# broadinstitute/delphy

Hardware: AMD Instinct MI355X
Metric: MCMC moves/sec on 100k-tip SARS-CoV-2 EMAT at 1/2/4/8 MI355X (higher is better)
Workload: dtype f64; 1 GPU; C4: synthetic 100000-tip EMAT, 29903 sites, HKY(kappa=5) + skygrid, 8092 partition parts (199999 nodes), 1000 moves/part/step, move mix 7.5/7.5/15/1/1; parts_per_gpu=8092, parts_requested=8192, max_part_nodes=-1, lds_staging=True, tickets_per_part_and_pass=4, parallelism=parts sharded over 1 GPU(s), one wavefront per part, collectives=none (one rank), emat_build_id=7d9b3896ecee7423

## Files before the change

delphy_amd/csrc/emat_device_core.hpp:

```cpp
#ifndef EMAT_DEV_NS
#error "define EMAT_DEV_NS and EMAT_VARIANT_LDS before including the device headers"
#endif

#include <hip/hip_runtime.h>
#include <cfloat>
#include <cstdint>

#include "emat_slab.hpp"

#ifndef EMAT_DEVICE_COMMON_ONCE_
#define EMAT_DEVICE_COMMON_ONCE_
namespace emat {
extern __shared__ __attribute__((aligned(16))) uint8_t emat_lds[];
constexpr uint32_t k_lds_tables_bytes = k_max_lds_partitions * (1 + 4 + 16) * 8;
constexpr uint32_t k_lds_ctx_bytes = 288;
#ifndef EMAT_RNG_BLOCKS
#define EMAT_RNG_BLOCKS 32
#endif
constexpr uint32_t k_rng_blocks = EMAT_RNG_BLOCKS;
static_assert(k_rng_blocks == 0 || (k_rng_blocks <= 64 && (k_rng_blocks & (k_rng_blocks - 1)) == 0), "one block per lane, a power of two");
constexpr uint32_t k_lds_rng_bytes = k_rng_blocks * 16;
constexpr uint32_t k_lds_static_bytes = k_lds_tables_bytes + k_lds_ctx_bytes + k_lds_rng_bytes + k_max_lds_partitions * 16 * 8;
__shared__ __attribute__((aligned(16))) uint8_t emat_lds_tables[k_lds_tables_bytes];
__shared__ __attribute__((aligned(16))) uint8_t emat_lds_ctx[k_lds_ctx_bytes];
// ... 497 lines not shown
  double r;
  { EMAT_TIMED(0);
    r = delta_lambda_across_node_missations_fresh(c, node); }
  *e = (uint64_t)__double_as_longlong(r);
  return r;
}
template <bool kMemo = true> EMAT_D double delta_lambda_across_branch(Ctx& c, int node) {
  double r = 0.0;
  const MutRec* m = muts_of(c, node); int nm = nmuts(c, node);
  for (int i = 0; i < nm; ++i) { int l = m[i].site; r += mu_of(c)[site_part(c, l)] * site_nu(c, l) * (q_a(c, l, m[i].to) - q_a(c, l, m[i].from)); }
  r += kMemo ? delta_lambda_across_node_missations(c, node) : delta_lambda_across_node_missations_fresh(c, node);
  return r;
}
EMAT_DN double calc_lambda_at_node(Ctx& c, int node) {
  double r = c.cumQ[c.L];
  for (int cur = node; cur != k_no_node; cur = nodes_of(c)[cur].parent) r += delta_lambda_across_branch(c, cur);
  return r;
}
EMAT_D double log_mu_nu_q(const Ctx& c, int l, int a, int b) {
  const int pa = site_part(c, l); const double nu = site_nu(c, l);
  if (c.have_logq && nu == 1.0) return emat_lds_logq[pa * 16 + a * 4 + b];
  return m_log(mu_of(c)[pa] * nu * q_of(c)[pa * 16 + a * 4 + b]);
}
EMAT_D double branch_log_G(const Ctx& c, double t_P, double t_X, double lambda_X, const MutRec* m, int nm) {
  double r = -lambda_X * (t_X - t_P);
  for (int i = nm - 1; i >= 0; --i) {
    int l = m[i].site;
    r -= mu_of(c)[site_part(c, l)] * site_nu(c, l) * (q_a(c, l, m[i].from) - q_a(c, l, m[i].to)) * (m[i].t - t_P);
    r += log_mu_nu_q(c, l, m[i].from, m[i].to);
  }
  return r;
}
EMAT_DN int calc_site_state_at(Ctx& c, int branch, double t, int l) {
  for (int cur = branch; cur != k_no_node; cur = nodes_of(c)[cur].parent) {
    const MutRec* m = muts_of(c, cur);
    for (int i = nmuts(c, cur) - 1; i >= 0; --i) { if (m[i].t > t) continue; if (m[i].site == l) return m[i].to; }
  }
  return c.ref[l];
}
EMAT_D bool is_site_missing_at(Ctx& c, int node, int l) {
  for (int cur = node; cur != k_no_node; cur = nodes_of(c)[cur].parent) if (miss_contains(c, cur, l)) return true;
  return false;
}
EMAT_DN SVec<IvRec> reconstruct_missing_sites_at(Ctx& c, int node) { EMAT_TIMED(0);
  int total = 0;
  for (int cur = node; cur != k_no_node; cur = nodes_of(c)[cur].parent) total += (int)nodes_of(c)[cur].miss.cnt;
  SVec<IvRec> a = sc_vec<IvRec>(c, total + 1), b = sc_vec<IvRec>(c, total + 1);
  if (c.failed) return a;
  IvRec* so_far = a.p; IvRec* other = b.p; int n = 0;
  for (int cur = node; cur != k_no_node; cur = nodes_of(c)[cur].parent) {
    const int cnt = (int)nodes_of(c)[cur].miss.cnt;
    if (cnt == 0) continue;
    int k = iv_merge(other, so_far, n, miss_of(c, cur), cnt);
    IvRec* t = so_far; so_far = other; other = t; n = k;
  }
  SVec<IvRec> r; r.p = so_far; r.n = n; r.cap = total + 1;
  return r;
}
EMAT_D bool descends_from(Ctx& c, int X, int A) {
  if (A == k_no_node) return true;
  for (int cur = X; cur != k_no_node; cur = nodes_of(c)[cur].parent) {
    if (cur == A) return true;
    if (nodes_of(c)[cur].t < nodes_of(c)[A].t) return false;
  }
  return false;
}
EMAT_DN int find_MRCA_of(Ctx& c, int P, int Q) {
  if (P == k_no_node) return P;
  if (Q == k_no_node) return Q;
  int guard = 0;
  while (P != Q && guard++ < (1 << 28)) {
    double tP = nodes_of(c)[P].t, tQ = nodes_of(c)[Q].t;
    if (tP > tQ) { P = nodes_of(c)[P].parent; EMAT_CHECK(c, P != k_no_node); if (P == k_no_node) return Q; }
    else if (tP < tQ) { Q = nodes_of(c)[Q].parent; EMAT_CHECK(c, Q != k_no_node); if (Q == k_no_node) return P; }
    else if (is_tip(c, P)) { P = nodes_of(c)[P].parent; if (P == k_no_node) return Q; }
    else if (is_tip(c, Q)) { Q = nodes_of(c)[Q].parent; if (Q == k_no_node) return P; }
    else {
      int dP = 0, dQ = 0;
      for (int x = P; x != k_no_node; x = nodes_of(c)[x].parent) ++dP;
      for (int x = Q; x != k_no_node; x = nodes_of(c)[x].parent) ++dQ;
      int a = P, b = Q;
      while (dP > dQ) { a = nodes_of(c)[a].parent; --dP; }
      while (dQ > dP) { b = nodes_of(c)[b].parent; --dQ; }
      while (a != b) { a = nodes_of(c)[a].parent; b = nodes_of(c)[b].parent; }
      return a;
    }
  }
  return P;
}

EMAT_DF int skygrid_interval(const PopTable& p, double t) {
  const int n = p.skygrid_num_knots;
  double g = (t - p.skygrid_x[0]) * p.skygrid_inv_dx;
  int k = g > 0.0 ? (g < (double)n ? (int)g : n) : 0;
  while (k > 0 && !(p.skygrid_x[k - 1] < t)) --k;
  while (k < n && p.skygrid_x[k] < t) ++k;
  return k;
}
EMAT_DF double skygrid_log_N(const PopTable& p, double t) {
  int k = skygrid_interval(p, t), M = p.skygrid_num_knots - 1;
  if (k == 0) return p.skygrid_gamma[0];
  if (k > M) return p.skygrid_gamma[M];
  if (p.skygrid_type == 1) return p.skygrid_gamma[k];
  double cc = (t - p.skygrid_x[k - 1]) / (p.skygrid_x[k] - p.skygrid_x[k - 1]);
  return (1 - cc) * p.skygrid_gamma[k - 1] + cc * p.skygrid_gamma[k];
}
EMAT_DF double pop_at_time(const PopTable& p, double t) {
  if (p.kind == 0) return p.p[0];
  if (p.kind == 1) { double v = p.p[1] * m_exp((t - p.p[0]) * p.p[2]); return p.p[3] > v ? p.p[3] : v; }
  return m_exp(skygrid_log_N(p, t));
}
EMAT_DF double uniform_f64(double v) {
  const uint64_t a = __builtin_bit_cast(uint64_t, v);
  const uint32_t lo = __builtin_amdgcn_readfirstlane((uint32_t)a), hi = __builtin_amdgcn_readfirstlane((uint32_t)(a >> 32));
  return __builtin_bit_cast(double, ((uint64_t)hi << 32) | lo);
}
EMAT_DF double skygrid_log_N_uniform(const EMAT_CONST_AS PopTable* p, double t) {
  const EMAT_CONST_AS double* x = uniform_const_ptr((const double*)p->skygrid_x);
  const EMAT_CONST_AS double* ga = uniform_const_ptr((const double*)p->skygrid_gamma);
  const int n = p->skygrid_num_knots, M = n - 1;
  const double g = (t - x[0]) * p->skygrid_inv_dx;
  int k = __builtin_amdgcn_readfirstlane(g > 0.0 ? (g < (double)n ? (int)g : n) : 0);
  while (k > 0 && !(x[k - 1] < t)) --k;
  while (k < n && x[k] < t) ++k;
  if (k == 0) return ga[0];
  if (k > M) return ga[M];
  if (p->skygrid_type == 1) return ga[k];
  const double cc = (t - x[k - 1]) / (x[k] - x[k - 1]);
  return (1 - cc) * ga[k - 1] + cc * ga[k];
}
EMAT_DF double log_pop_ratio_uniform(const PopTable* pp, double t_new, double t_old) {
  const EMAT_CONST_AS PopTable* p = uniform_const_ptr(pp);
  const int kind = p->kind;
  if (kind == 0) return 0.0;
  t_new = uniform_f64(t_new); t_old = uniform_f64(t_old);
  if (kind == 2) return skygrid_log_N_uniform(p, t_new) - skygrid_log_N_uniform(p, t_old);
  const double t0 = p->p[0], n0 = p->p[1], gr = p->p[2], floor_n = p->p[3];
  double a = n0 * m_exp((t_new - t0) * gr); a = floor_n > a ? floor_n : a;
  double b = n0 * m_exp((t_old - t0) * gr); b = floor_n > b ? floor_n : b;
  return m_log(a / b);
}
EMAT_D double exp_unclamped_int(const PopTable& p, double a, double b) { double n0 = p.p[1], g = p.p[2], t0 = p.p[0]; return n0 / g * m_exp(g * (a - t0)) * m_expm1(g * (b - a)); }
EMAT_DN double skygrid_log_int_N(const PopTable& p, double a, double b) {
  const double* x = p.skygrid_x; const double* ge = p.skygrid_gamma;
  int M = p.skygrid_num_knots - 1;
  int ka = skygrid_interval(p, a), kb = skygrid_interval(p, b);
  int kka = ka - 1 > 0 ? ka - 1 : 0, kkb = kb < M ? kb : M;
  double bias = -k_inf;
  for (int k = kka; k <= kkb; ++k) bias = bias > ge[k] ? bias : ge[k];
  double result = 0.0;
  for (int k = ka; k <= kb; ++k) {
    double lo = k > 0 ? (a > x[k - 1] ? a : x[k - 1]) : a;
    double hi = k <= M ? (b < x[k] ? b : x[k]) : b;
    if (k == 0) result += m_exp(-bias + ge[0]) * (hi - lo);
    else if (k == M + 1) result += m_exp(-bias + ge[M]) * (hi - lo);
    else if (p.skygrid_type == 1) result += m_exp(-bias + ge[k]) * (hi - lo);
    else if (ge[k] == ge[k - 1]) result += m_exp(-bias + ge[k]) * (hi - lo);
    else {
      double c_lo = (lo - x[k - 1]) / (x[k] - x[k - 1]), c_hi = (hi - x[k - 1]) / (x[k] - x[k - 1]);
      double G_lo = (1 - c_lo) * ge[k - 1] + c_lo * ge[k], G_hi = (1 - c_hi) * ge[k - 1] + c_hi * ge[k];
      double D = G_hi - G_lo;
      if (D == 0.0) result += m_exp(-bias + G_lo) * (hi - lo);
      else result += m_exp(-bias + G_lo) * (hi - lo) * (m_expm1(D) / D);
    }
  }
  return m_log(result) + bias;
}
EMAT_NOTAIL EMAT_DN double pop_integral(const PopTable& p, double a, double b) {
  if (p.kind == 0) return (b - a) * p.p[0];
  if (p.kind == 1) {
    double n0 = p.p[1], g = p.p[2], t0 = p.p[0], min_pop = p.p[3], t_c = p.t_c;
    if (min_pop == 0.0) return g == 0.0 ? (b - a) * n0 : exp_unclamped_int(p, a, b);
    if (g == 0.0) return (b - a) * (min_pop > n0 ? min_pop : n0);
    if (g > 0.0) {
      if (b <= t_c) return (b - a) * min_pop;
      if (a >= t_c) return exp_unclamped_int(p, a, b);
      return (t_c - a) * min_pop + n0 / g * m_exp(g * (t_c - t0)) * m_expm1(g * (b - t_c));
    }
    if (a >= t_c) return (b - a) * min_pop;
    if (b <= t_c) return exp_unclamped_int(p, a, b);
    return n0 / g * m_exp(g * (a - t0)) * m_expm1(g * (t_c - a)) + (b - t_c) * min_pop;
  }
  return m_exp(skygrid_log_int_N(p, a, b));
}
EMAT_D double exp_unclamped_intensity(const PopTable& p, double a, double b) { double n0 = p.p[1], g = p.p[2], t0 = p.p[0]; return -1.0 / (n0 * g) * m_exp(-g * (a - t0)) * m_expm1(-g * (b - a)); }
EMAT_DN double skygrid_log_int_inv_N(const PopTable& p, double a, double b) {
  const double* x = p.skygrid_x; const double* gm = p.skygrid_gamma;
  int M = p.skygrid_num_knots - 1;
  int ka = skygrid_interval(p, a), kb = skygrid_interval(p, b);
  int kka = ka - 1 > 0 ? ka - 1 : 0, kkb = kb < M ? kb : M;
  double bias = -k_inf;
  for (int k = kka; k <= kkb; ++k) bias = bias > -gm[k] ? bias : -gm[k];
  double result = 0.0;
  for (int k = ka; k <= kb; ++k) {
    double lo = k > 0 ? (a > x[k - 1] ? a : x[k - 1]) : a;
    double hi = k <= M ? (b < x[k] ? b : x[k]) : b;
    if (k == 0) result += m_exp(-bias + -gm[0]) * (hi - lo);
    else if (k == M + 1) result += m_exp(-bias + -gm[M]) * (hi - lo);
    else if (p.skygrid_type == 1) result += m_exp(-bias + -gm[k]) * (hi - lo);
    else if (gm[k] == gm[k - 1]) result += m_exp(-bias + -gm[k]) * (hi - lo);
    else {
      double c_lo = (lo - x[k - 1]) / (x[k] - x[k - 1]), c_hi = (hi - x[k - 1]) / (x[k] - x[k - 1]);
      double G_lo = (1 - c_lo) * -gm[k - 1] + c_lo * -gm[k], G_hi = (1 - c_hi) * -gm[k - 1] + c_hi * -gm[k];
      double D = G_hi - G_lo;
      if (D == 0.0) result += m_exp(-bias + G_lo) * (hi - lo);
      else result += m_exp(-bias + G_lo) * (hi - lo) * (m_expm1(D) / D);
    }
  }
  return m_log(result) + bias;
}
EMAT_NOTAIL EMAT_DN double pop_intensity_integral(const PopTable& p, double a, double b) {
  if (p.kind == 0) return (b - a) / p.p[0];
  if (p.kind == 1) {
    double n0 = p.p[1], g = p.p[2], t0 = p.p[0], min_pop = p.p[3], t_c = p.t_c;
    if (min_pop == 0.0) return g == 0.0 ? (b - a) / n0 : exp_unclamped_intensity(p, a, b);
    if (g == 0.0) return (b - a) / (min_pop > n0 ? min_pop : n0);
    double inv_min_pop = 1.0 / min_pop;
    if (g > 0.0) {
      if (b <= t_c) return (b - a) * inv_min_pop;
      if (a >= t_c) return exp_unclamped_intensity(p, a, b);
      return (t_c - a) * inv_min_pop - 1.0 / (n0 * g) * m_exp(-g * (t_c - t0)) * m_expm1(-g * (b - t_c));
    }
    if (a >= t_c) return (b - a) * inv_min_pop;
    if (b <= t_c) return exp_unclamped_intensity(p, a, b);
    return -1.0 / (n0 * g) * m_exp(-g * (a - t0)) * m_expm1(-g * (t_c - a)) + (b - t_c) * inv_min_pop;
  }
  return m_exp(skygrid_log_int_inv_N(p, a, b));
}

struct Cells {
  double* kbar_p; double* ktw_p;
  double* ktw; double* popsize; double* ts_over_pop; int32_t* nactive;
  const EMAT_CONST_AS double* sh_ktw; const EMAT_CONST_AS double* sh_tsop; const EMAT_CONST_AS int32_t* sh_nact;
  int first; bool local;
};
EMAT_D Cells cells_of(Ctx& c) {
  Cells k; const int cap = hdr_of(c)->cell_cap;
  double* base = (double*)slab_at(c, hdr_of(c)->off_cells);
  k.kbar_p = base; k.ktw_p = base + cap; k.first = hdr_of(c)->cell_first; k.local = c.includes_run_root;
  if (k.local) { k.ktw = base + 2 * cap; k.popsize = base + 3 * cap; k.ts_over_pop = base + 4 * cap; k.nactive = (int32_t*)(base + 5 * cap); k.sh_ktw = nullptr; k.sh_tsop = nullptr; k.sh_nact = nullptr; }
  else { k.ktw = nullptr; k.popsize = nullptr; k.ts_over_pop = nullptr; k.nactive = nullptr; k.sh_ktw = uniform_const_ptr(c.sh_ktw); k.sh_tsop = uniform_const_ptr(c.sh_tsop); k.sh_nact = uniform_const_ptr(c.sh_nact); }
  return k;
}
EMAT_D int cell_for(const Ctx& c, double t) { return (int)floor((hdr_of(c)->t_ref - t) / hdr_of(c)->t_step); }
EMAT_D double cell_ubound(const Ctx& c, int cell) { return hdr_of(c)->t_ref - hdr_of(c)->t_step * cell; }
EMAT_D double cell_lbound(const Ctx& c, int cell) { return cell_ubound(c, cell) - hdr_of(c)->t_step; }
EMAT_NOTAIL EMAT_DN void coal_grow(Ctx& c, int cell);
template <bool kGrow = true> EMAT_DF void coal_ensure_space(Ctx& c, double t) {
  int cell = cell_for(c, t);
  if (kGrow) { if (cell >= hdr_of(c)->n_cells_total && c.includes_run_root) coal_grow(c, cell); }
  if (cell < hdr_of(c)->cell_first || cell >= hdr_of(c)->n_cells_total) EMAT_FAIL(c, k_part_internal);
}
EMAT_NOTAIL EMAT_DN void coal_grow(Ctx& c, int cell) {
  {
    Cells k = cells_of(c);
    while (hdr_of(c)->n_cells_total <= cell) {
      int i = hdr_of(c)->n_cells_total, w = i - hdr_of(c)->cell_first;
      if (w >= hdr_of(c)->cell_cap) { EMAT_FAIL(c, k_part_cell_overflow); return; }
      double popsize_bar_i = pop_integral(*c.pop, cell_lbound(c, i), cell_ubound(c, i)) / hdr_of(c)->t_step;
      double sigma = sqrt(popsize_bar_i / hdr_of(c)->t_step);
      double ktw = gaussian(c, 0.0, sigma);
      k.popsize[w] = popsize_bar_i; k.ts_over_pop[w] = hdr_of(c)->t_step / popsize_bar_i; k.nactive[w] = 1; k.kbar_p[w] = 1.0; k.ktw_p[w] = ktw; k.ktw[w] = ktw;
      hdr_of(c)->n_cells_total = i + 1; hdr_of(c)->n_cells = w + 1;
    }
  }
}
EMAT_DF bool coal_needs_cells(const Ctx& c, double t) {
  if (!c.includes_run_root) return false;
  const int cell = cell_for(c, t);
  return cell >= hdr_of(c)->n_cells_total && cell - hdr_of(c)->cell_first >= hdr_of(c)->cell_cap;
}
EMAT_DN void stop_for_cells(Ctx& c, int kind) {
  rng_rewind_to_move_start(c);
  hdr_of(c)->proposed[kind]--;
  c.failed = true;
  if (hdr_of(c)->status == 0) hdr_of(c)->status = k_part_need_cells;
}
EMAT_DF void coal_add_interval(Ctx& c, double t_start, double t_end, double delta_k) {
  if (c.failed) return;
  if (t_start < t_end) { double t = t_start; t_start = t_end; t_end = t; }
  Cells k = cells_of(c);
  const int first = hdr_of(c)->cell_first;
  int cell_start = cell_for(c, t_start);
  int cell_end = hdr_of(c)->n_cells_total - 1;
  if (t_end != cell_lbound(c, cell_end)) cell_end = cell_for(c, t_end);
  if (cell_start < first || cell_end >= hdr_of(c)->n_cells_total || cell_start > cell_end) { EMAT_FAIL(c, k_part_internal); return; }
  const double ts = hdr_of(c)->t_step;
  if (cell_start == cell_end) k.kbar_p[cell_start - first] += delta_k * (t_start - t_end) / ts;
  else {
    k.kbar_p[cell_start - first] += delta_k * (t_start - cell_lbound(c, cell_start)) / ts;
    k.kbar_p[cell_end - first] += delta_k * (cell_ubound(c, cell_end) - t_end) / ts;
    for (int i = cell_start + 1; i < cell_end; ++i) k.kbar_p[i - first] += delta_k;
  }
  c.bytes += 8 * (int64_t)(cell_end - cell_start + 1); c.bytes_w += 8 * (int64_t)(cell_end - cell_start + 1);
}
EMAT_DF double coal_cell_term(const Ctx& c, const Cells& k, int w, double new_k, double old_k) {
  double na, tsop, ktw;
  if (k.local) { na = (double)k.nactive[w]; tsop = k.ts_over_pop[w]; ktw = k.ktw[w]; }
  else { const int i = __builtin_amdgcn_readfirstlane(k.first + w); na = (double)k.sh_nact[i]; tsop = k.sh_tsop[i]; ktw = k.sh_ktw[i]; }
  return tsop * (
      +0.5 * (new_k * new_k - old_k * old_k) * na
      - (k.ktw_p[w] * na - ktw + 0.5) * (new_k - old_k));
}
template <bool kGrow = true> EMAT_DF double coal_delta_on_add_interval(Ctx& c, double min_t, double max_t, double delta_k) { EMAT_TIMED(0);
  { int cm = cell_for(c, max_t); if (cm < hdr_of(c)->cell_first || cm >= hdr_of(c)->n_cells_total) { EMAT_FAIL(c, k_part_internal); return 0.0; } }
  coal_ensure_space<kGrow>(c, min_t);
  if (c.failed) return 0.0;
  if (min_t == max_t) return 0.0;
  Cells k = cells_of(c);
  const int first = hdr_of(c)->cell_first; const double ts = hdr_of(c)->t_step;
  int cell_start = cell_for(c, max_t), cell_end = cell_for(c, min_t);
  double d = 0.0;
  if (cell_start == cell_end) {
    int w = cell_start - first;
    double old_k = k.kbar_p[w], new_k = old_k + delta_k * (max_t - min_t) / ts;
    d -= coal_cell_term(c, k, w, new_k, old_k);
  } else {
    int i = cell_start;
    double dt_start = max_t - cell_lbound(c, cell_start);
    double dt_end = cell_ubound(c, cell_end) - min_t;
    double old_k = k.kbar_p[i - first], new_k = old_k + delta_k * dt_start / ts;
    d -= coal_cell_term(c, k, i - first, new_k, old_k);
    for (++i; i < cell_end; ++i) { old_k = k.kbar_p[i - first]; new_k = old_k + delta_k; d -= coal_cell_term(c, k, i - first, new_k, old_k); }
    old_k = k.kbar_p[i - first]; new_k = old_k + delta_k * dt_end / ts;
    d -= coal_cell_term(c, k, i - first, new_k, old_k);
  }
  c.bytes += 36 * (int64_t)(cell_end - cell_start + 1);
  EMAT_COUNT(c, 13, cell_end - cell_start + 1); EMAT_COUNT(c, 14, 1);
  return d;
}
template <bool kGrow = true> EMAT_DF double coal_delta_displace_coalescence(Ctx& c, double old_t, double new_t) { EMAT_TIMED(0);
  double d = (old_t <= new_t) ? coal_delta_on_add_interval<kGrow>(c, old_t, new_t, -1.0) : coal_delta_on_add_interval<kGrow>(c, new_t, old_t, +1.0);
  { EMAT_TIMED(0); d -= log_pop_ratio_uniform(c.pop, new_t, old_t); }
  return d;
}
template <bool kGrow = true> EMAT_DF double coal_delta_displace_tip(Ctx& c, double old_t, double new_t) {
  return (old_t <= new_t) ? coal_delta_on_add_interval<kGrow>(c, old_t, new_t, +1.0) : coal_delta_on_add_interval<kGrow>(c, new_t, old_t, -1.0);
}
template <bool kGrow = true> EMAT_DF void coal_coalescence_displaced(Ctx& c, double old_t, double new_t) {
  coal_ensure_space<kGrow>(c, new_t);
  coal_add_interval(c, old_t, new_t, old_t <= new_t ? -1.0 : +1.0);
}
template <bool kGrow = true> EMAT_DF void coal_tip_displaced(Ctx& c, double old_t, double new_t) {
  coal_ensure_space<kGrow>(c, new_t);
  coal_add_interval(c, old_t, new_t, old_t <= new_t ? +1.0 : -1.0);
}

EMAT_DN double gamma_q_fraction(double a, double x) {
  const double FPMIN = 1e-300;
  double b = x + 1.0 - a, cc = 1.0 / FPMIN, d = 1.0 / b, h = d;
  for (int i = 1; i < 100000; ++i) {
    double an = -i * (i - a);
    b += 2.0;
    d = an * d + b; if (fabs(d) < FPMIN) d = FPMIN;
    cc = b + an / cc; if (fabs(cc) < FPMIN) cc = FPMIN;
    d = 1.0 / d;
    double del = d * cc; h *= del;
    if (fabs(del - 1.0) < 1e-16) break;
  }
  return h;
}
EMAT_DN double gamma_q(double a, double x) {
  if (x == 0.0) return 1.0;
  if (isinf(x)) return 0.0;
  const double lg = lgamma(a);
  if (x < a + 1.0) {
    double ap = a, sum = 1.0 / a, del = sum;
    for (int n = 0; n < 100000; ++n) { ap += 1.0; del *= x / ap; sum += del; if (fabs(del) < fabs(sum) * 1e-17) break; }
    return 1.0 - sum * m_exp(-x + a * m_log(x) - lg);
  }
  return m_exp(-x + a * m_log(x) - lg) * gamma_q_fraction(a, x);
}
EMAT_DN double gamma_q_inv(double a, double q) {
  if (q == 0.0) return k_inf;
  if (q == 1.0) return 0.0;
  const double lg = lgamma(a);
  if (q < 1e-3) {
    const double lq = m_log(q);
    double x = a + 1.0, h = gamma_q_fraction(a, x), prev = 0.0;
    if (-x + a * m_log(x) - lg + m_log(h) > lq) {
      for (int j = 0; j < 100; ++j) {
        double dx = (-x + a * m_log(x) - lg + m_log(h) - lq) * x * h;
        double xn = x + dx;
        if (xn < a + 1.0) xn = a + 1.0;
        bool done = fabs(xn - x) <= 1e-14 * xn || (j > 2 && fabs(dx) >= fabs(prev));
        x = xn; prev = dx;
        if (done) break;
        h = gamma_q_fraction(a, x);
      }
      return x;
    }
  }
  const double p = 1.0 - q;
  double x;
  if (a > 1.0) {
    double pp = (p < 0.5) ? p : q;
    double t = sqrt(-2.0 * m_log(pp));
    double xg = (2.30753 + t * 0.27061) / (1.0 + t * (0.99229 + t * 0.04481)) - t;
    if (p < 0.5) xg = -xg;
    double v = a * pow(1.0 - 1.0 / (9.0 * a) - xg / (3.0 * sqrt(a)), 3.0);
    x = v > 1e-3 ? v : 1e-3;
  } else {
    double t = 1.0 - a * (0.253 + a * 0.12);
    if (p < t) x = pow(p / t, 1.0 / a);
    else x = 1.0 - m_log(1.0 - (p - t) / (1.0 - t));
  }
  const double a1 = a - 1.0;
  for (int j = 0; j < 60; ++j) {
    if (x <= 0.0) x = 1e-300;
    double err = gamma_q(a, x) - q;
    double tdens = m_exp(-x + a1 * m_log(x) - lg);
    if (tdens == 0.0) break;
    double u = -err / tdens;
    double w = u * (a1 / x - 1.0);
    double dx = u / (1.0 - 0.5 * (w < 1.0 ? w : 1.0));
    double xn = x - dx;
    if (xn <= 0.0) xn = 0.5 * x;
    double tol = 1e-15 * (xn > 1e-300 ? xn : 1e-300);
    if (fabs(xn - x) < tol) { x = xn; break; }
    x = xn;
  }
  return x;
}

}
}
```

delphy_amd/csrc/emat_device_moves.hpp:

```cpp

#include "emat_device_spr.hpp"

namespace emat {
namespace EMAT_DEV_NS {

#ifndef EMAT_HOT_BYTES
#define EMAT_HOT_BYTES 1536
#endif
enum { k_inner_node_displace = 0, k_tip_displace = 1, k_branch_reform = 2, k_subtree_slide = 3, k_spr1 = 4 };

EMAT_D void begin_move(Ctx& c, int kind) { hdr_of(c)->proposed[kind]++; c.tr_kind = (double)kind; c.tr_node = -1.0; c.tr_acc = 0.0; c.tr_log_mh = __builtin_nan(""); }
EMAT_D void note_move(Ctx& c, int node, double log_mh, bool acc, int kind) { c.tr_node = (double)node; c.tr_log_mh = log_mh; c.tr_acc = acc ? 1.0 : 0.0; if (acc) hdr_of(c)->accepted[kind]++; }
EMAT_D bool mh_accept(Ctx& c, double log_mh) { return log_mh >= 0.0 || uniform_co(c, 0.0, 1.0) < m_exp(log_mh); }

EMAT_DF double bounded_exponential(Ctx& c, double lambda, double a, double b) {
  double u = u01_oo(c);
  double ltr = lambda * (b - a);
  double x;
  if (lambda == 0.0) x = a + u * (b - a);
  else if (lambda > 0 && ltr > 100) x = b + m_log(u) / lambda;
  else if (lambda < 0 && ltr < -100) x = a + m_log(u) / lambda;
  else x = a + m_log1p(u * (m_exp(ltr) - 1)) / lambda;
  return x < a ? a : (b < x ? b : x);
}
EMAT_DF int pick_random_node(Ctx& c) { return uniform_int(c, hdr_of(c)->n_nodes); }

struct CoreFrame {
  int X, new_branch, P, old_S;
  double new_t, alpha_ratio, old_t_P, d_prior, log_mh;
  Graft old_graft, new_graft;
};
#ifndef EMAT_CF
#define EMAT_CF(c) (*(CoreFrame*)(c).frame)
#endif
EMAT_NOTAIL EMAT_DN void spr_move_core(Ctx& c, int X, int new_branch, double new_t, double alpha_ratio) { EMAT_TIMED(2);
  if (X == hdr_of(c)->root) return;
  if (!c.includes_run_root) if (nodes_of(c)[X].parent == hdr_of(c)->root || new_branch == hdr_of(c)->root) return;
  {
    const double t_X = nodes_of(c)[X].t;
    const int P = nodes_of(c)[X].parent;
    const double new_t_P = new_t;
    if (new_t_P == t_X || new_t_P == nodes_of(c)[new_branch].t || (P != hdr_of(c)->root && new_t_P == nodes_of(c)[nodes_of(c)[P].parent].t)) return;
    if (coal_needs_cells(c, new_t_P)) { stop_for_cells(c, (int)c.tr_kind); return; }
    CoreFrame* f = (CoreFrame*)sc_alloc(c, (uint32_t)sizeof(CoreFrame));
    if (c.failed) return;
    c.frame = (uint8_t*)f;
    f->X = X; f->new_branch = new_branch; f->P = P; f->old_S = sibling_of(c, P, X);
    f->new_t = new_t; f->alpha_ratio = alpha_ratio; f->old_t_P = nodes_of(c)[P].t;
  }
  c.mu_prop = nodes_of(c)[hdr_of(c)->root].lambda / (c.L - nodes_of(c)[hdr_of(c)->root].n_missing);
  EMAT_PHASE_BEGIN();
  analyze_graft(c, EMAT_CF(c).X, EMAT_CF(c).old_graft);
  peel_graft(c, EMAT_CF(c).old_graft);
  EMAT_PHASE(c, 0);
  spr_move_topology(c, EMAT_CF(c).X, EMAT_CF(c).new_branch, EMAT_CF(c).new_t);
  EMAT_PHASE(c, 1);
  propose_new_graft(c, EMAT_CF(c).X, EMAT_CF(c).new_graft);
  EMAT_PHASE(c, 2);
  if (c.failed) return;
  EMAT_CF(c).d_prior = coal_delta_displace_coalescence(c, EMAT_CF(c).old_t_P, EMAT_CF(c).new_t);
  {
    const CoreFrame& f = EMAT_CF(c);
    EMAT_CF(c).log_mh = (f.new_graft.delta_log_G - f.new_graft.log_alpha_mut) - (f.old_graft.delta_log_G - f.old_graft.log_alpha_mut) + m_log(f.alpha_ratio) + f.d_prior;
  }
  if (c.failed) return;
  const bool acc = mh_accept(c, EMAT_CF(c).log_mh);
  if (c.tr_kind == (double)k_subtree_slide) note_move(c, EMAT_CF(c).X, EMAT_CF(c).log_mh, acc, k_subtree_slide);
  if (acc) {
    apply_graft(c, EMAT_CF(c).new_graft);
    hdr_of(c)->log_G -= EMAT_CF(c).old_graft.delta_log_G; hdr_of(c)->log_G += EMAT_CF(c).new_graft.delta_log_G;
    hdr_of(c)->log_aug_prior += EMAT_CF(c).d_prior;
    coal_coalescence_displaced(c, EMAT_CF(c).old_t_P, EMAT_CF(c).new_t);
  } else {
    spr_move_topology(c, EMAT_CF(c).X, EMAT_CF(c).old_S, EMAT_CF(c).old_t_P);
    apply_graft(c, EMAT_CF(c).old_graft);
  }
  EMAT_PHASE(c, 4);
}

template <bool kRoot> EMAT_NOTAIL EMAT_DN void inner_node_displace_move(Ctx& c) { EMAT_TIMED(2);
  begin_move(c, k_inner_node_displace);
  int node;
  { EMAT_TIMED(2);
    int guard = 0; do { node = pick_random_node(c); } while (is_tip(c, node) && guard++ < (1 << 26)); }
  c.tr_node = (double)node;
  const int root = hdr_of(c)->root;
  if (!kRoot && node == root) return;
  const NodeRec nd = nodes_of(c)[node];
  double t_min = -k_inf;
  if (!kRoot || node != root) {
    t_min = nodes_of(c)[nd.parent].t;
    const MutRec* m = muts_of(c, node);
    for (int i = 0; i < (int)nd.muts.cnt; ++i) t_min = t_min > m[i].t ? t_min : m[i].t;
  }
  double t_max = k_inf;
  const int ch[2] = {nd.child0, nd.child1};
  const double lambda_at_node = nd.lambda;
  double d_logG_dt = 0.0;
  if (!kRoot || node != root) d_logG_dt += -lambda_at_node;
  for (int k = 0; k < 2; ++k) {
    const int cc = ch[k];
    t_max = t_max < nodes_of(c)[cc].t ? t_max : nodes_of(c)[cc].t;
    const MutRec* m = muts_of(c, cc);
    const int nm = nmuts(c, cc);
    for (int i = 0; i < nm; ++i) t_max = t_max < m[i].t ? t_max : m[i].t;
    c.bytes += 64 + 16 * nm + 24 * (int)nodes_of(c)[cc].miss.cnt;
  }
  { EMAT_TIMED(2);
  for (int k = 0; k < 2; ++k) {
    double lambda_just_below = lambda_at_node + delta_lambda_across_node_missations(c, ch[k]);
    d_logG_dt -= -lambda_just_below;
  } }
  c.bytes += 2 * 64 + 16 * (int)nd.muts.cnt;
  const double old_t = nd.t;
  double log_alpha_ratio = 0.0, new_t = old_t;
  if (kRoot && node == root) {
    double tree_span = c.t_max_tip - t_max;
    EMAT_CHECK(c, tree_span >= 0.0);
    double ds = (1 / nd.lambda) / 2;
    double delta_scale;
    if (tree_span < ds) delta_scale = tree_span; else delta_scale = ds;
    new_t = old_t + gaussian(c, 0.0, delta_scale);
    if (new_t < t_min || new_t > t_max) return;
    log_alpha_ratio = 0.0;
  } else {
    EMAT_TIMED(2);
    new_t = bounded_exponential(c, d_logG_dt, t_min, t_max);
    log_alpha_ratio = d_logG_dt * (new_t - old_t);
  }
  if (new_t == t_min || new_t == t_max) return;
  if (kRoot) { if (coal_needs_cells(c, new_t)) { stop_for_cells(c, k_inner_node_displace); return; } }
  double delta_log_G = d_logG_dt * (new_t - old_t);
  double delta_log_prior = coal_delta_displace_coalescence<kRoot>(c, old_t, new_t);
  if (c.failed) return;
  double log_mh = delta_log_G + delta_log_prior - log_alpha_ratio;
  bool acc;
  { EMAT_TIMED(2);
  acc = mh_accept(c, log_mh);
  note_move(c, node, log_mh, acc, k_inner_node_displace); }
  if (acc) {
    EMAT_TIMED(2);
    coal_coalescence_displaced<kRoot>(c, old_t, new_t);
    nodes_of(c)[node].t = new_t;
    hdr_of(c)->log_G += d_logG_dt * (new_t - old_t);
    hdr_of(c)->log_aug_prior += delta_log_prior;
  }
}

template <bool kRoot> EMAT_NOTAIL EMAT_DN void tip_displace_move(Ctx& c) { EMAT_TIMED(2);
  begin_move(c, k_tip_displace);
  int node;
  { int guard = 0; do { node = pick_random_node(c); } while (!is_tip(c, node) && guard++ < (1 << 26)); }
  c.tr_node = (double)node;
  const NodeRec nd = nodes_of(c)[node];
  if (nd.t_min == nd.t_max) return;
  double t_min;
  if ((double)nd.t_min < nodes_of(c)[nd.parent].t) t_min = nodes_of(c)[nd.parent].t; else t_min = (double)nd.t_min;
  const MutRec* m = muts_of(c, node);
  for (int i = 0; i < (int)nd.muts.cnt; ++i) t_min = t_min > m[i].t ? t_min : m[i].t;
  const double t_max = (double)nd.t_max;
  const double d_logG_dt = -nd.lambda;
  const double old_t = nd.t;
  c.bytes += 2 * 64 + 16 * (int)nd.muts.cnt;
  double new_t = bounded_exponential(c, d_logG_dt, t_min, t_max);
  double log_alpha_ratio = d_logG_dt * (new_t - old_t);
  if (new_t == t_min || new_t == t_max) return;
  double delta_log_G = d_logG_dt * (new_t - old_t);
  double delta_log_prior = coal_delta_displace_tip<kRoot>(c, old_t, new_t);
  if (c.failed) return;
  double log_mh = delta_log_G + delta_log_prior - log_alpha_ratio;
  bool acc = mh_accept(c, log_mh);
  note_move(c, node, log_mh, acc, k_tip_displace);
  if (acc) {
    coal_tip_displaced<kRoot>(c, old_t, new_t);
    nodes_of(c)[node].t = new_t;
    hdr_of(c)->log_G += d_logG_dt * (new_t - old_t);
    hdr_of(c)->log_aug_prior += delta_log_prior;
  }
}

EMAT_DF SVec<MutRec> randomize_branch_mutation_times(Ctx& c, int X) { EMAT_TIMED(2);
  const int n = nmuts(c, X);
  SVec<MutRec> out = sc_vec<MutRec>(c, n);
  if (c.failed) return out;
  const MutRec* old = muts_of(c, X);
  if (X == hdr_of(c)->root) { for (int i = 0; i < n; ++i) push(c, out, old[i]); return out; }
  const double t_X = nodes_of(c)[X].t, t_P = nodes_of(c)[nodes_of(c)[X].parent].t;
  bool complicated = false;
  for (int i = 0; i < n && !complicated; ++i) for (int j = i + 1; j < n; ++j) if (old[i].site == old[j].site) { complicated = true; break; }
  if (!complicated) {
    for (int i = 0; i < n; ++i) { MutRec r = make_mut(old[i].from, old[i].site, old[i].to, uniform_oc(c, t_P, t_X)); r.pad = (uint16_t)i; push(c, out, r); }
  } else {
    int prev_site = -1;
    while (true) {
      int l = 0x7fffffff;
      for (int i = 0; i < n; ++i) if (old[i].site > prev_site && old[i].site < l) l = old[i].site;
      if (l == 0x7fffffff) break;
      prev_site = l;
      int first = out.n, k = 0;
      for (int i = 0; i < n; ++i) if (old[i].site == l) { MutRec r = make_mut(old[i].from, old[i].site, old[i].to, uniform_oc(c, t_P, t_X)); r.pad = (uint16_t)i; push(c, out, r); ++k; }
      for (int a = first + 1; a < first + k && a < out.n; ++a) { double x = out.p[a].t; int b = a - 1; while (b >= first && out.p[b].t > x) { out.p[b + 1].t = out.p[b].t; --b; } out.p[b + 1].t = x; }
    }
  }
  sort_muts(out.p, out.n);
  return out;
}

struct ReformFactors { double* A; double* B; };
EMAT_DF ReformFactors reform_factors(Ctx& c, const MutRec* m, int n) { EMAT_TIMED(2);
  ReformFactors f; f.A = (double*)sc_alloc(c, (uint32_t)n * 16u); f.B = f.A + n;
  if (c.failed) return f;
  uint32_t need_log = 0u; bool all_logs = false;
  for (int j0 = 0; j0 < n; j0 += 4) {
    int l[4]; int pa[4]; double nu[4];
#pragma unroll
    for (int k = 0; k < 4; ++k) l[k] = m[j0 + k < n ? j0 + k : n - 1].site;
#pragma unroll
    for (int k = 0; k < 4; ++k) { pa[k] = site_part(c, l[k]); nu[k] = site_nu(c, l[k]); }
#pragma unroll
    for (int k = 0; k < 4; ++k) if (j0 + k < n) {
      const MutRec& mm = m[j0 + k];
      const double mn = mu_of(c)[pa[k]] * nu[k];
      const double* q = q_of(c) + pa[k] * 16;
      f.A[j0 + k] = mn * (-q[(int)mm.from * 5] - -q[(int)mm.to * 5]);
      if (c.have_logq && nu[k] == 1.0) f.B[j0 + k] = emat_lds_logq[pa[k] * 16 + (int)mm.from * 4 + (int)mm.to];
      else { f.B[j0 + k] = mn * q[(int)mm.from * 4 + (int)mm.to]; need_log |= 1u << ((j0 + k) & 31); if (j0 + k >= 32) all_logs = true; }
    }
  }
  if (all_logs) { for (int j = 0; j < n; ++j) if (!(c.have_logq && site_nu(c, m[j].site) == 1.0)) f.B[j] = m_log(f.B[j]); }
  else if (need_log != 0u) { const int n32 = n < 32 ? n : 32; for (int j = 0; j < n32; ++j) if ((need_log >> j) & 1u) f.B[j] = m_log(f.B[j]); }
  return f;
}
template <bool kRoot> EMAT_NOTAIL EMAT_DN void branch_reform_move(Ctx& c) { EMAT_TIMED(2);
  begin_move(c, k_branch_reform);
  if (hdr_of(c)->n_nodes < 3) return;
  const int X = pick_random_node(c);
  c.tr_node = (double)X;
  if (X == hdr_of(c)->root) return;
  const int P = nodes_of(c)[X].parent;
  const int S = sibling_of(c, P, X);
  const double t_X = nodes_of(c)[X].t, t_P = nodes_of(c)[P].t;
  if (kRoot) { if (P == hdr_of(c)->root) { spr_move_core(c, X, S, t_P, 1.0); if (c.failed) return; } }
  const double lam = nodes_of(c)[X].lambda;
  const int n = nmuts(c, X);
  if (n == 0) {
    const double g = -lam * (t_X - t_P), delta_log_G = g - g;
    c.bytes += 2 * 64;
    const bool acc = mh_accept(c, delta_log_G);
    note_move(c, X, delta_log_G, acc, k_branch_reform);
    if (acc) hdr_of(c)->log_G += delta_log_G;
    return;
  }
  const ReformFactors f = reform_factors(c, muts_of(c, X), n);
  SVec<MutRec> nm = randomize_branch_mutation_times(c, X);
  if (c.failed) return;
  double g_new = -lam * (t_X - t_P), g_old = g_new;
  { const MutRec* m = nm.p; for (int i = nm.n - 1; i >= 0; --i) { const int j = (int)m[i].pad; g_new -= f.A[j] * (m[i].t - t_P); g_new += f.B[j]; } }
  { const MutRec* m = muts_of(c, X); for (int i = n - 1; i >= 0; --i) { g_old -= f.A[i] * (m[i].t - t_P); g_old += f.B[i]; } }
  const double delta_log_G = g_new - g_old;
  c.bytes += 2 * 64 + 2 * 16 * nm.n;
  double log_mh = delta_log_G;
  bool acc = mh_accept(c, log_mh);
  note_move(c, X, log_mh, acc, k_branch_reform);
  if (acc) {
    for (int i = 0; i < nm.n; ++i) nm.p[i].pad = 0;
    list_assign<MutRec>(c, nodes_of(c)[X].muts, nm.p, nm.n); hdr_of(c)->log_G += delta_log_G; c.bytes += 16 * nm.n; c.bytes_w += 16 * nm.n;
  }
}

EMAT_DN SVec<int> enumerate_descendant_branches_straddling(Ctx& c, int P, double t, int X) {
  SVec<int> out; out.n = 0;
  ScSpan span = sc_span(c, 512);
  out.p = (int*)span.lo; out.cap = 0;
  int* stack_base = (int*)span.hi;
  int sp = 0;
  auto room = [&](int er, int es) -> bool {
    if (span.lo + (size_t)(out.n + er) * 4 + 16 <= span.hi - (size_t)(sp + es) * 4) return true;
    if (!span.lds) return false;
    ScSpan big = sc_span_hbm(c);
    if (big.lo + (size_t)(out.n + er) * 4 + 16 > big.hi - (size_t)(sp + es) * 4) return false;
    int* no = (int*)big.lo; int* nb = (int*)big.hi;
    for (int i = 0; i < out.n; ++i) no[i] = out.p[i];
    for (int i = 1; i <= sp; ++i) nb[-i] = stack_base[-i];
    span = big; out.p = no; stack_base = nb;
    return true;
  };
  if (!room(0, 1)) { EMAT_FAIL(c, k_part_overflow); return out; }
  stack_base[-(++sp)] = P;
  while (sp > 0 && !c.failed) {
    int n = stack_base[-sp]; --sp;
    if (n == X) continue;
    if (t <= nodes_of(c)[n].t) { if (!room(1, 0)) { EMAT_FAIL(c, k_part_overflow); break; } out.p[out.n++] = n; }
    else if (!is_tip(c, n)) {
      if (!room(0, 2)) { EMAT_FAIL(c, k_part_overflow); break; }
      stack_base[-(++sp)] = nodes_of(c)[n].child1;
      stack_base[-(++sp)] = nodes_of(c)[n].child0;
    }
  }
  out.cap = out.n;
  sc_span_commit(c, span, (uint32_t)out.n * 4u);
  return out;
}

EMAT_NOTAIL EMAT_DN void subtree_slide_move(Ctx& c) { EMAT_TIMED(2);
  begin_move(c, k_subtree_slide);
  if (hdr_of(c)->n_nodes < 2) return;
  const int X = pick_random_node(c);
  c.tr_node = (double)X;
  const int root = hdr_of(c)->root;
  if (X == root) return;
  const int P = nodes_of(c)[X].parent, S = sibling_of(c, P, X);
  double t_early = (P == root) ? (nodes_of(c)[X].t < nodes_of(c)[S].t ? nodes_of(c)[X].t : nodes_of(c)[S].t) : nodes_of(c)[root].t;
  if (P == root) { if (nodes_of(c)[S].t < nodes_of(c)[X].t) t_early = nodes_of(c)[S].t; else t_early = nodes_of(c)[X].t; }
  double tree_span = c.t_max_tip - t_early;
  EMAT_CHECK(c, tree_span >= 0.0);
  double ds = (1 / nodes_of(c)[X].lambda) / 2;
  double delta_scale = tree_span < ds ? tree_span : ds;
  double delta_t = gaussian(c, 0.0, delta_scale);
  const double old_P_t = nodes_of(c)[P].t, new_P_t = old_P_t + delta_t;
  if (delta_t < 0.0) {
    if (P != root && new_P_t < nodes_of(c)[nodes_of(c)[P].parent].t) {
      int GG = nodes_of(c)[P].parent, SS = P;
      while (new_P_t < nodes_of(c)[GG].t) { SS = GG; GG = nodes_of(c)[GG].parent; if (GG == k_no_node) break; }
      SVec<int> branches = enumerate_descendant_branches_straddling(c, SS, old_P_t, X);
      if (c.failed) return;
      double a_o2n = 1.0, a_n2o = 1.0 / (double)branches.n;
      spr_move_core(c, X, SS, new_P_t, a_n2o / a_o2n);
    } else spr_move_core(c, X, S, new_P_t, 1.0);
  } else {
    if (new_P_t > nodes_of(c)[X].t) return;
    if (new_P_t > nodes_of(c)[S].t) {
      SVec<int> branches = enumerate_descendant_branches_straddling(c, P, new_P_t, X);
      if (c.failed) return;
      if (branches.n == 0) return;
      int bi = uniform_int(c, branches.n);
      int SS = branches.p[bi];
      double a_o2n = 1.0 / (double)branches.n, a_n2o = 1.0;
      spr_move_core(c, X, SS, new_P_t, a_n2o / a_o2n);
    } else spr_move_core(c, X, S, new_P_t, 1.0);
  }
}

EMAT_D void spr1_park(Ctx& c, int phase) { c.phase = (uint8_t)phase; c.svc = 1; }
EMAT_NOTAIL EMAT_DN void spr1_move_begin(Ctx& c) { EMAT_TIMED(2);
  begin_move(c, k_spr1);
  c.phase = 0;
  if (hdr_of(c)->n_nodes < 2) return;
  const double chooser = uniform_co(c, 0.0, 1.0);
  const int limit = chooser < 0.01 ? 0x7fffffff : 1;
  const int root0 = hdr_of(c)->root;
  c.mu_prop = nodes_of(c)[root0].lambda / (c.L - nodes_of(c)[root0].n_missing);
  int X;
  { int guard = 0; do { X = pick_random_node(c); } while (hdr_of(c)->root == X && guard++ < (1 << 26)); }
  c.tr_node = (double)X;
  if (nodes_of(c)[X].lambda == 0.0) return;
  const int P = nodes_of(c)[X].parent;
  const bool pruning_changes_root = P == hdr_of(c)->root;
  if (pruning_changes_root && !c.includes_run_root) return;
  EMAT_PHASE_BEGIN();
  Spr1Frame* frp = (Spr1Frame*)sc_alloc(c, (uint32_t)sizeof(Spr1Frame));
  if (c.failed) return;
  Spr1Frame& fr = *frp;
  c.frame = (uint8_t*)frp;
  fr.X = X; fr.t_X = nodes_of(c)[X].t; fr.P = P; fr.old_t_P = nodes_of(c)[P].t; fr.old_S = sibling_of(c, P, X); fr.old_G = nodes_of(c)[P].parent;
  fr.limit = limit; fr.f = 0.8 ; fr.t_max_tip = c.t_max_tip; fr.can_change_root = c.includes_run_root;
  {
    const uint32_t a0 = (c.a_top + 15u) & ~15u, free_b = c.a_end > a0 ? c.a_end - a0 : 0u;
    uint32_t hot_b = EMAT_HOT_BYTES;
    if (free_b / 2 > hot_b) hot_b = (free_b / 2 < 32768u ? free_b / 2 : 32768u) & ~15u;
    fr.hot = (limit == 1) ? sc_reserve_hot(c, hot_b) : HotBlock{nullptr, 0};
  }
  analyze_graft(c, X, fr.old_graft);
  peel_graft(c, fr.old_graft);
  EMAT_PHASE(c, 5);
  if (c.failed) return;
  fr.old_min_muts = count_min_mutations(c, fr.old_graft);
  int extra = 4;
  if (limit != 1) { extra = 8; for (int n = 0; n < hdr_of(c)->n_nodes; ++n) if (c.includes_run_root || n != hdr_of(c)->root) extra += nmuts(c, n); }
  fr.extra = extra;
  fr.deltas = summarize_closed_mutations(c, fr.old_graft, extra);
  fr.missing_at_X = reconstruct_missing_sites_at(c, X);
  fr.n_missing_at_X = iv_num_sites(fr.missing_at_X.p, fr.missing_at_X.n);
  fr.lambda_X = nodes_of(c)[X].lambda;
  fr.init_branch = fr.old_S;
  if (c.failed) return;
  spr1_park(c, 1);
}
EMAT_NOTAIL EMAT_DN void spr1_move_propose(Ctx& c) { EMAT_TIMED(2);
  Spr1Frame& fr = *(Spr1Frame*)c.frame;
  c.phase = 0;
  if (c.failed) return;
  EMAT_PHASE_BEGIN();
  const Study& pre = fr.study;
  const int X = fr.X, P = fr.P;
  int new_region; double new_t_P;
  { EMAT_TIMED(2);
  new_region = study_pick_nexus_region(c, pre);
  new_t_P = study_pick_time_in_region(c, pre, new_region);
  fr.log_alpha_o2n = study_log_alpha_in_region(c, pre, new_region, new_t_P); }
  const int new_S = pre.regions.p[new_region].branch;
  EMAT_CHECK(c, new_S != P);
  fr.pre_new_region_min_muts = pre.regions.p[new_region].min_muts;
  fr.new_S = new_S; fr.new_t_P = new_t_P;
  const double t_new_S = nodes_of(c)[new_S].t;
  int new_G = nodes_of(c)[new_S].parent;
  if (new_G == P) new_G = fr.old_G;
  const double t_new_G = (new_G == k_no_node) ? k_neg_dbl_max : nodes_of(c)[new_G].t;
  if (c.failed) return;
  EMAT_PHASE(c, 7);
  if (new_t_P == fr.t_X || new_t_P == t_new_S || new_t_P == t_new_G) { apply_graft(c, fr.old_graft); return; }
  if (coal_needs_cells(c, new_t_P)) { apply_graft(c, fr.old_graft); if (!c.failed) stop_for_cells(c, k_spr1); return; }
  spr_move_topology(c, X, new_S, new_t_P);
  EMAT_PHASE(c, 8);
  propose_new_graft(c, X, fr.new_graft);
  EMAT_PHASE(c, 9);
  if (c.failed) return;
  EMAT_CHECK(c, nodes_of(c)[X].parent == P);
  fr.new_min_muts = count_min_mutations(c, fr.new_graft);
  fr.deltas = summarize_closed_mutations(c, fr.new_graft, fr.extra);
  fr.init_branch = new_S;
  if (c.failed) return;
  spr1_park(c, 2);
}
EMAT_NOTAIL EMAT_DN void spr1_move_finish(Ctx& c) { EMAT_TIMED(2);
  Spr1Frame& fr = *(Spr1Frame*)c.frame;
  c.phase = 0;
  if (c.failed) return;
  EMAT_PHASE_BEGIN();
  const Study& post = fr.study;
  const int X = fr.X;
  const int old_region = study_find_region(post, fr.old_S, fr.old_t_P);
  EMAT_CHECK(c, old_region != -1);
  if (c.failed) return;
  const double log_alpha_n2o = study_log_alpha_in_region(c, post, old_region, fr.old_t_P);
  EMAT_CHECK(c, fr.new_min_muts == fr.pre_new_region_min_muts);
  EMAT_CHECK(c, fr.old_min_muts == post.regions.p[old_region].min_muts);
  EMAT_PHASE(c, 11);
  const double d_prior = coal_delta_displace_coalescence(c, fr.old_t_P, fr.new_t_P);
  if (c.failed) return;
  const double log_mh = (fr.new_graft.delta_log_G - fr.new_graft.log_alpha_mut) - (fr.old_graft.delta_log_G - fr.old_graft.log_alpha_mut)
      + log_alpha_n2o - fr.log_alpha_o2n + d_prior;
  const bool acc = mh_accept(c, log_mh);
  note_move(c, X, log_mh, acc, k_spr1);
  if (acc) {
    apply_graft(c, fr.new_graft);
    hdr_of(c)->log_G -= fr.old_graft.delta_log_G; hdr_of(c)->log_G += fr.new_graft.delta_log_G;
    hdr_of(c)->log_aug_prior += d_prior;
    coal_coalescence_displaced(c, fr.old_t_P, fr.new_t_P);
  } else {
    EMAT_TIMED(2);
    spr_move_topology(c, X, fr.old_S, fr.old_t_P);
    apply_graft(c, fr.old_graft);
  }
  EMAT_PHASE(c, 12);
}

EMAT_DN bool compact_heap(Ctx& c) {
  uint32_t live = 0;
  const int n = hdr_of(c)->n_nodes;
  for (int i = 0; i < n; ++i) {
    live += (((uint32_t)nodes_of(c)[i].muts.cnt * 16u) + 15u) & ~15u;
    live += (((uint32_t)nodes_of(c)[i].miss.cnt * 8u) + 15u) & ~15u;
    live += (((uint32_t)nodes_of(c)[i].mfs.cnt * 8u) + 15u) & ~15u;
  }
  if (live > hdr_of(c)->scratch_end - hdr_of(c)->scratch_begin) return false;
  uint8_t* stage = c.G + hdr_of(c)->scratch_begin;
  uint32_t w = 0;
  for (int i = 0; i < n; ++i) {
    ListRef* refs[3] = {&nodes_of(c)[i].muts, &nodes_of(c)[i].miss, &nodes_of(c)[i].mfs};
    const uint32_t es[3] = {16u, 8u, 8u};
    for (int k = 0; k < 3; ++k) {
      uint32_t bytes = (uint32_t)refs[k]->cnt * es[k];
      const uint64_t* src = (const uint64_t*)heap_at(c, refs[k]->off); uint64_t* dst = (uint64_t*)(stage + w);
      for (uint32_t q = 0; q < bytes / 8; ++q) dst[q] = src[q];
      w += (bytes + 15u) & ~15u;
    }
  }
// ... 105 lines not shown
```

Baseline: 485.9 million moves/s.

## Reuse coalescent span values on accept and bound exp in MH test

```diff
diff --git a/delphy_amd/csrc/emat_device_core.hpp b/delphy_amd/csrc/emat_device_core.hpp
--- a/delphy_amd/csrc/emat_device_core.hpp
+++ b/delphy_amd/csrc/emat_device_core.hpp
@@ -823,46 +823,72 @@
       +0.5 * (new_k * new_k - old_k * old_k) * na
       - (k.ktw_p[w] * na - ktw + 0.5) * (new_k - old_k));
 }
-template <bool kGrow = true> EMAT_DF double coal_delta_on_add_interval(Ctx& c, double min_t, double max_t, double delta_k) { EMAT_TIMED(0);
-  { int cm = cell_for(c, max_t); if (cm < hdr_of(c)->cell_first || cm >= hdr_of(c)->n_cells_total) { EMAT_FAIL(c, k_part_internal); return 0.0; } }
-  coal_ensure_space<kGrow>(c, min_t);
-  if (c.failed) return 0.0;
-  if (min_t == max_t) return 0.0;
+struct CoalSpan { double d; double k_start, k_end; int w_start, w_end; bool apply; };
+template <bool kGrow = true> EMAT_DF CoalSpan coal_span_on_add_interval(Ctx& c, double min_t, double max_t, double delta_k) { EMAT_TIMED(0);
+  CoalSpan sp; sp.d = 0.0; sp.k_start = sp.k_end = 0.0; sp.w_start = sp.w_end = 0; sp.apply = false;
+  const int first = hdr_of(c)->cell_first;
+  const int cell_start = cell_for(c, max_t);
+  if (cell_start < first || cell_start >= hdr_of(c)->n_cells_total) { EMAT_FAIL(c, k_part_internal); return sp; }
+  const int cell_end = cell_for(c, min_t);
+  if (kGrow) { if (cell_end >= hdr_of(c)->n_cells_total && c.includes_run_root) coal_grow(c, cell_end); }
+  const int total = hdr_of(c)->n_cells_total;
+  if (cell_end < first || cell_end >= total) EMAT_FAIL(c, k_part_internal);
+  if (c.failed) return sp;
+  if (min_t == max_t) return sp;
   Cells k = cells_of(c);
-  const int first = hdr_of(c)->cell_first; const double ts = hdr_of(c)->t_step;
-  int cell_start = cell_for(c, max_t), cell_end = cell_for(c, min_t);
+  const double ts = hdr_of(c)->t_step;
   double d = 0.0;
   if (cell_start == cell_end) {
     int w = cell_start - first;
     double old_k = k.kbar_p[w], new_k = old_k + delta_k * (max_t - min_t) / ts;
     d -= coal_cell_term(c, k, w, new_k, old_k);
+    sp.k_start = sp.k_end = new_k;
   } else {
     int i = cell_start;
     double dt_start = max_t - cell_lbound(c, cell_start);
     double dt_end = cell_ubound(c, cell_end) - min_t;
     double old_k = k.kbar_p[i - first], new_k = old_k + delta_k * dt_start / ts;
     d -= coal_cell_term(c, k, i - first, new_k, old_k);
+    sp.k_start = new_k;
     for (++i; i < cell_end; ++i) { old_k = k.kbar_p[i - first]; new_k = old_k + delta_k; d -= coal_cell_term(c, k, i - first, new_k, old_k); }
     old_k = k.kbar_p[i - first]; new_k = old_k + delta_k * dt_end / ts;
     d -= coal_cell_term(c, k, i - first, new_k, old_k);
+    sp.k_end = new_k;
   }
   c.bytes += 36 * (int64_t)(cell_end - cell_start + 1);
   EMAT_COUNT(c, 13, cell_end - cell_start + 1); EMAT_COUNT(c, 14, 1);
-  return d;
-}
-template <bool kGrow = true> EMAT_DF double coal_delta_displace_coalescence(Ctx& c, double old_t, double new_t) { EMAT_TIMED(0);
-  double d = (old_t <= new_t) ? coal_delta_on_add_interval<kGrow>(c, old_t, new_t, -1.0) : coal_delta_on_add_interval<kGrow>(c, new_t, old_t, +1.0);
-  { EMAT_TIMED(0); d -= log_pop_ratio_uniform(c.pop, new_t, old_t); }
-  return d;
-}
-template <bool kGrow = true> EMAT_DF double coal_delta_displace_tip(Ctx& c, double old_t, double new_t) {
-  return (old_t <= new_t) ? coal_delta_on_add_interval<kGrow>(c, old_t, new_t, +1.0) : coal_delta_on_add_interval<kGrow>(c, new_t, old_t, -1.0);
+  sp.d = d; sp.w_start = cell_start - first; sp.w_end = cell_end - first;
+  sp.apply = cell_end == total - 1 || min_t != cell_lbound(c, total - 1);
+  return sp;
+}
+template <bool kGrow = true> EMAT_DF double coal_delta_on_add_interval(Ctx& c, double min_t, double max_t, double delta_k) { return coal_span_on_add_interval<kGrow>(c, min_t, max_t, delta_k).d; }
+EMAT_DF void coal_apply_span(Ctx& c, const CoalSpan sp, double delta_k) {
+  double* kbar_p = (double*)slab_at(c, hdr_of(c)->off_cells);
+  kbar_p[sp.w_start] = sp.k_start;
+  if (sp.w_start != sp.w_end) {
+    kbar_p[sp.w_end] = sp.k_end;
+    for (int w = sp.w_start + 1; w < sp.w_end; ++w) kbar_p[w] += delta_k;
+  }
+  c.bytes += 8 * (int64_t)(sp.w_end - sp.w_start + 1); c.bytes_w += 8 * (int64_t)(sp.w_end - sp.w_start + 1);
+}
+template <bool kGrow = true> EMAT_DF CoalSpan coal_span_displace_coalescence(Ctx& c, double old_t, double new_t) { EMAT_TIMED(0);
+  CoalSpan sp = (old_t <= new_t) ? coal_span_on_add_interval<kGrow>(c, old_t, new_t, -1.0) : coal_span_on_add_interval<kGrow>(c, new_t, old_t, +1.0);
+  { EMAT_TIMED(0); sp.d -= log_pop_ratio_uniform(c.pop, new_t, old_t); }
+  return sp;
+}
+template <bool kGrow = true> EMAT_DF double coal_delta_displace_coalescence(Ctx& c, double old_t, double new_t) { return coal_span_displace_coalescence<kGrow>(c, old_t, new_t).d; }
+template <bool kGrow = true> EMAT_DF CoalSpan coal_span_displace_tip(Ctx& c, double old_t, double new_t) {
+  return (old_t <= new_t) ? coal_span_on_add_interval<kGrow>(c, old_t, new_t, +1.0) : coal_span_on_add_interval<kGrow>(c, new_t, old_t, -1.0);
 }
 template <bool kGrow = true> EMAT_DF void coal_coalescence_displaced(Ctx& c, double old_t, double new_t) {
   coal_ensure_space<kGrow>(c, new_t);
   coal_add_interval(c, old_t, new_t, old_t <= new_t ? -1.0 : +1.0);
 }
-template <bool kGrow = true> EMAT_DF void coal_tip_displaced(Ctx& c, double old_t, double new_t) {
+template <bool kGrow = true> EMAT_DF void coal_coalescence_displaced(Ctx& c, const CoalSpan sp, double old_t, double new_t) {
+  if (sp.apply) coal_apply_span(c, sp, old_t <= new_t ? -1.0 : +1.0); else coal_coalescence_displaced<kGrow>(c, old_t, new_t);
+}
+template <bool kGrow = true> EMAT_DF void coal_tip_displaced(Ctx& c, const CoalSpan sp, double old_t, double new_t) {
+  if (sp.apply) { coal_apply_span(c, sp, old_t <= new_t ? +1.0 : -1.0); return; }
   coal_ensure_space<kGrow>(c, new_t);
   coal_add_interval(c, old_t, new_t, old_t <= new_t ? +1.0 : -1.0);
 }
diff --git a/delphy_amd/csrc/emat_device_moves.hpp b/delphy_amd/csrc/emat_device_moves.hpp
--- a/delphy_amd/csrc/emat_device_moves.hpp
+++ b/delphy_amd/csrc/emat_device_moves.hpp
@@ -11,7 +11,14 @@
 
 EMAT_D void begin_move(Ctx& c, int kind) { hdr_of(c)->proposed[kind]++; c.tr_kind = (double)kind; c.tr_node = -1.0; c.tr_acc = 0.0; c.tr_log_mh = __builtin_nan(""); }
 EMAT_D void note_move(Ctx& c, int node, double log_mh, bool acc, int kind) { c.tr_node = (double)node; c.tr_log_mh = log_mh; c.tr_acc = acc ? 1.0 : 0.0; if (acc) hdr_of(c)->accepted[kind]++; }
-EMAT_D bool mh_accept(Ctx& c, double log_mh) { return log_mh >= 0.0 || uniform_co(c, 0.0, 1.0) < m_exp(log_mh); }
+EMAT_D bool mh_accept(Ctx& c, double log_mh) {
+  if (log_mh >= 0.0) return true;
+  const double u = uniform_co(c, 0.0, 1.0);
+  const double y = -log_mh, y2 = y * y;
+  if (u * ((1.0 + y) + y2 * (0.5 + y * (1.0 / 6.0))) > 1.0 + 0x1p-40 && u >= 0x1p-1000) return false;
+  if (y < 1.0 && u < ((1.0 - y) + y2 * (0.5 - y * (1.0 / 6.0))) - 0x1p-40) return true;
+  return u < m_exp(log_mh);
+}
 
 EMAT_DF double bounded_exponential(Ctx& c, double lambda, double a, double b) {
   double u = u01_oo(c);
@@ -131,8 +138,9 @@
   if (new_t == t_min || new_t == t_max) return;
   if (kRoot) { if (coal_needs_cells(c, new_t)) { stop_for_cells(c, k_inner_node_displace); return; } }
   double delta_log_G = d_logG_dt * (new_t - old_t);
-  double delta_log_prior = coal_delta_displace_coalescence<kRoot>(c, old_t, new_t);
-  if (c.failed) return;
+  const CoalSpan span = coal_span_displace_coalescence<kRoot>(c, old_t, new_t);
+  if (c.failed) return;
+  const double delta_log_prior = span.d;
   double log_mh = delta_log_G + delta_log_prior - log_alpha_ratio;
   bool acc;
   { EMAT_TIMED(2);
@@ -140,7 +148,7 @@
   note_move(c, node, log_mh, acc, k_inner_node_displace); }
   if (acc) {
     EMAT_TIMED(2);
-    coal_coalescence_displaced<kRoot>(c, old_t, new_t);
+    coal_coalescence_displaced<kRoot>(c, span, old_t, new_t);
     nodes_of(c)[node].t = new_t;
     hdr_of(c)->log_G += d_logG_dt * (new_t - old_t);
     hdr_of(c)->log_aug_prior += delta_log_prior;
@@ -166,13 +174,14 @@
   double log_alpha_ratio = d_logG_dt * (new_t - old_t);
   if (new_t == t_min || new_t == t_max) return;
   double delta_log_G = d_logG_dt * (new_t - old_t);
-  double delta_log_prior = coal_delta_displace_tip<kRoot>(c, old_t, new_t);
-  if (c.failed) return;
+  const CoalSpan span = coal_span_displace_tip<kRoot>(c, old_t, new_t);
+  if (c.failed) return;
+  const double delta_log_prior = span.d;
   double log_mh = delta_log_G + delta_log_prior - log_alpha_ratio;
   bool acc = mh_accept(c, log_mh);
   note_move(c, node, log_mh, acc, k_tip_displace);
   if (acc) {
-    coal_tip_displaced<kRoot>(c, old_t, new_t);
+    coal_tip_displaced<kRoot>(c, span, old_t, new_t);
     nodes_of(c)[node].t = new_t;
     hdr_of(c)->log_G += d_logG_dt * (new_t - old_t);
     hdr_of(c)->log_aug_prior += delta_log_prior;
```

New measurement: 497.9 million moves/s, median of 6. +2.5%, better.
